# mims-harvard/Raindrop

Measured on AMD Instinct MI355X. Metric: samples/sec fwd+bwd, P19 34-sensor batch=256; % HBM roofline on msg-pass kernel, higher is better.
Workload: dtype f32

## Files before the change

### raindrop_amd/csrc/rd_attnfuse.hip

```cpp
#include <stdlib.h>

#include "rd_common.h"
#include "rd_plan.h"
#include "rd_rng.h"

namespace rd {
namespace {

typedef __bf16 bf8 __attribute__((ext_vector_type(8)));
typedef __bf16 bf4 __attribute__((ext_vector_type(4)));
typedef short sh4 __attribute__((ext_vector_type(4)));
typedef short sh8 __attribute__((ext_vector_type(8)));

constexpr int TS = 64;
constexpr int LDT = TS;
__device__ __forceinline__ int tsw(int row) { return (row & 3) | (((row >> 3) & 1) << 2); }
__device__ __forceinline__ int tofs(int row, int col) { return row * LDT + ((((col >> 3) ^ tsw(row)) & 7) << 3) + (col & 7); }
constexpr int AF_WV = 8, AF_THR = 64 * AF_WV;

struct FAttnArgs {
  const float* x;
  const __bf16* wf;
  const __bf16* wb;
  const float* bias;
  float* out; float* lse;
  const float* dout; const float* ds1; float* dx;
  __bf16* xt; __bf16* dt;
  const int32_t* plan;
  int T, B, D, H, hd;
  float scale, p_drop; uint64_t seed; uint32_t site; const uint64_t* seed_cell;
  int one;
  unsigned long long* stamps;
};
static unsigned long long* g_af_stamps = nullptr;
#define AFSTAMP(i)                                                                                  \
  do {                                                                                              \
    if (a.stamps && blockIdx.x == 0 && threadIdx.x == 0) a.stamps[(i)] = clock64();                 \
  } while (0)

__device__ __forceinline__ float g16_max(float v) {
#define RD_ROR(v, n) __builtin_bit_cast(float, __builtin_amdgcn_update_dpp(0, __builtin_bit_cast(int, v), 0x120 + (n), 0xf, 0xf, false))
  v = fmaxf(v, RD_ROR(v, 8)); v = fmaxf(v, RD_ROR(v, 4)); v = fmaxf(v, RD_ROR(v, 2)); v = fmaxf(v, RD_ROR(v, 1));
  return v;
}
__device__ __forceinline__ float g16_sum(float v) {
  v += RD_ROR(v, 8); v += RD_ROR(v, 4); v += RD_ROR(v, 2); v += RD_ROR(v, 1);
#undef RD_ROR
  return v;
}

__device__ __forceinline__ bf8 frag_n(const __bf16* P, int ld, int row0, int k0, int lane) {
  return *reinterpret_cast<const bf8*>(P + (row0 + (lane & 15)) * ld + k0 + 8 * (lane >> 4));
}
__device__ __forceinline__ bf8 frag_t(const __bf16* P, int ld, int k0, int col0, int lane) {
  const int i = lane & 15, G = lane >> 4;
  const __bf16* src = P + (k0 + 8 * G + (i >> 2)) * ld + col0 + 4 * (i & 3);
  const sh4 lo = __builtin_amdgcn_ds_read_tr16_b64_v4i16((sh4 __attribute__((address_space(3)))*)(src));
  const sh4 hi = __builtin_amdgcn_ds_read_tr16_b64_v4i16((sh4 __attribute__((address_space(3)))*)(src + 4 * ld));
  const sh8 o = {lo[0], lo[1], lo[2], lo[3], hi[0], hi[1], hi[2], hi[3]};
  return __builtin_bit_cast(bf8, o);
}
__device__ __forceinline__ bf8 frag_ns(const __bf16* P, int row0, int k0, int lane) {
  return *reinterpret_cast<const bf8*>(P + tofs(row0 + (lane & 15), k0 + 8 * (lane >> 4)));
}
__device__ __forceinline__ bf8 frag_ts(const __bf16* P, int k0, int col0, int lane) {
  const int i = lane & 15, G = lane >> 4;
  const int row = k0 + 8 * G + (i >> 2), col = col0 + 4 * (i & 3);
  const __bf16* src = P + tofs(row, col);
  const sh4 lo = __builtin_amdgcn_ds_read_tr16_b64_v4i16((sh4 __attribute__((address_space(3)))*)(src));
  const sh4 hi = __builtin_amdgcn_ds_read_tr16_b64_v4i16((sh4 __attribute__((address_space(3)))*)(src + 4 * LDT));
  const sh8 o = {lo[0], lo[1], lo[2], lo[3], hi[0], hi[1], hi[2], hi[3]};
  return __builtin_bit_cast(bf8, o);
}
template <int NT, bool AT, bool BT, bool ASW, bool BSW>
__device__ __forceinline__ void mma_b16(f32x4 (&acc)[NT], const __bf16* Ah, const __bf16* Al, int lda, int a0, const __bf16* Bh,
                                        const __bf16* Bl, int ldb, int b0, int KK, int lane, bool one) {
  auto fa = [&](const __bf16* P, int k0) {
    if (ASW) return AT ? frag_ts(P, k0, a0, lane) : frag_ns(P, a0, k0, lane);
    return AT ? frag_t(P, lda, k0, a0, lane) : frag_n(P, lda, a0, k0, lane);
  };
  auto fb = [&](const __bf16* P, int k0, int j) {
    if (BSW) return BT ? frag_ts(P, k0, b0 + 16 * j, lane) : frag_ns(P, b0 + 16 * j, k0, lane);
    return BT ? frag_t(P, ldb, k0, b0 + 16 * j, lane) : frag_n(P, ldb, b0 + 16 * j, k0, lane);
  };
  if (!one) {
#pragma unroll
    for (int k0 = 0; k0 < KK; k0 += 32) {
      const bf8 ah = fa(Ah, k0);
      const bf8 al = fa(Al, k0);
      bf8 bh[NT], bl[NT];
#pragma unroll
      for (int j = 0; j < NT; ++j) { bh[j] = fb(Bh, k0, j); bl[j] = fb(Bl, k0, j); }
#pragma unroll
      for (int j = 0; j < NT; ++j) acc[j] = __builtin_amdgcn_mfma_f32_16x16x32_bf16(al, bh[j], acc[j], 0, 0, 0);
#pragma unroll
      for (int j = 0; j < NT; ++j) acc[j] = __builtin_amdgcn_mfma_f32_16x16x32_bf16(ah, bl[j], acc[j], 0, 0, 0);
#pragma unroll
      for (int j = 0; j < NT; ++j) acc[j] = __builtin_amdgcn_mfma_f32_16x16x32_bf16(ah, bh[j], acc[j], 0, 0, 0);
    }
  } else {
#pragma unroll
    for (int k0 = 0; k0 < KK; k0 += 32) {
      const bf8 ah = fa(Ah, k0);
#pragma unroll
      for (int j = 0; j < NT; ++j) {
        const bf8 bh = fb(Bh, k0, j);
        acc[j] = __builtin_amdgcn_mfma_f32_16x16x32_bf16(ah, bh, acc[j], 0, 0, 0);
      }
    }
  }
}

__device__ __forceinline__ void split4(const float (&v)[4], bf4& hi, bf4& lo) {
#pragma unroll
  for (int r = 0; r < 4; ++r) { hi[r] = (__bf16)v[r]; lo[r] = (__bf16)(v[r] - (float)hi[r]); }
}
__device__ __forceinline__ void store_t4(__bf16* Ph, __bf16* Pl, int row, int col4, const float (&v)[4]) {
  bf4 hi, lo;
  split4(v, hi, lo);
  const int o = tofs(row, col4);
  *reinterpret_cast<bf4*>(Ph + o) = hi;
  *reinterpret_cast<bf4*>(Pl + o) = lo;
}

__device__ __forceinline__ uint64_t attn_quad(int bh, int T, int q, int key) { return ((uint64_t)bh * T + key) * ((T + 3) >> 2) + (q >> 2); }
__device__ __forceinline__ void attn_keep4(float (&k4)[4], uint64_t seed, uint32_t site, int bh, int T, int q0, int key, float p, float inv_keep) {
  const float4 u = uniform4(seed, site, attn_quad(bh, T, q0, key));
  k4[0] = u.x >= p ? inv_keep : 0.f; k4[1] = u.y >= p ? inv_keep : 0.f;
  k4[2] = u.z >= p ? inv_keep : 0.f; k4[3] = u.w >= p ? inv_keep : 0.f;
}

template <int KCX>
struct XRows { float4 v[(TS * 8 * KCX) / AF_THR]; };

template <int KCX>
__device__ __forceinline__ void x_request(XRows<KCX>& r, const float* x, long row0, int Tv, int D, int tid) {
  constexpr int kq = 8 * KCX, NIT = (TS * kq) / AF_THR;
  static_assert((TS * kq) % AF_THR == 0, "x tile must divide over the workgroup");
#pragma unroll
  for (int it = 0; it < NIT; ++it) {
    const int i = tid + it * AF_THR;
    const int rr = i / kq, k = 4 * (i - rr * kq);
    r.v[it] = *reinterpret_cast<const float4*>(x + (row0 + min(rr, Tv - 1)) * D + min(k, D - 4));
  }
}
template <int KCX>
__device__ __forceinline__ void x_store(const XRows<KCX>& r, __bf16* Xh, __bf16* Xl, int Tv, int D, int tid) {
  constexpr int kq = 8 * KCX, NIT = (TS * kq) / AF_THR, LDX = 32 * KCX + 16;
#pragma unroll
  for (int it = 0; it < NIT; ++it) {
    const int i = tid + it * AF_THR;
    const int rr = i / kq, k = 4 * (i - rr * kq);
    const bool ok = rr < Tv && k < D;
    const float v[4] = {ok ? r.v[it].x : 0.f, ok ? r.v[it].y : 0.f, ok ? r.v[it].z : 0.f, ok ? r.v[it].w : 0.f};
    bf4 hi, lo;
    split4(v, hi, lo);
    *reinterpret_cast<bf4*>(Xh + rr * LDX + k) = hi;
    *reinterpret_cast<bf4*>(Xl + rr * LDX + k) = lo;
  }
}

template <int KCX>
struct QkvPanel { bf8 h[2][KCX], l[2][KCX]; float bs[2]; };

template <int NTH, int KCX>
__device__ __forceinline__ void qkv_request(QkvPanel<KCX>& p, const __bf16* wf_h, const float* bias, int D, int hd, int h, int wave, int lane) {
  constexpr int NCT3 = 3 * NTH;
  static_assert(NCT3 <= 2 * AF_WV, "two column tiles per wave");
#pragma unroll
  for (int s = 0; s < 2; ++s) {
    const int ct = min(wave + AF_WV * s, NCT3 - 1);
    const __bf16* t = wf_h + (size_t)ct * (KCX * 2 * 512) + lane * 8;
#pragma unroll
    for (int kc = 0; kc < KCX; ++kc) {
      p.h[s][kc] = *reinterpret_cast<const bf8*>(t + (kc * 2 + 0) * 512);
      p.l[s][kc] = *reinterpret_cast<const bf8*>(t + (kc * 2 + 1) * 512);
    }
    const int whc = ct / NTH, cl = 16 * (ct - whc * NTH) + (lane & 15);
    p.bs[s] = bias[whc * D + h * hd + min(cl, hd - 1)];
  }
}

template <int NTH, int KCX>
__device__ __forceinline__ void qkv_project(const QkvPanel<KCX>& p, const __bf16* Xh, const __bf16* Xl, int hd, int Tv, __bf16* Tp, int wave,
                                            int lane, bool one) {
  constexpr int NCT3 = 3 * NTH, HDP = 32 * ((16 * NTH + 31) / 32), LDX = 32 * KCX + 16;
  const bool two = wave + AF_WV < NCT3;
  const int aoff = (lane & 15) * LDX + 8 * (lane >> 4);
  f32x4 acc[2][4];
#pragma unroll
  for (int s = 0; s < 2; ++s)
#pragma unroll
    for (int rt = 0; rt < 4; ++rt) acc[s][rt] = (f32x4){0.f, 0.f, 0.f, 0.f};
  if (!one) {
#pragma unroll
    for (int kc = 0; kc < KCX; ++kc) {
      bf8 ah[4], al[4];
#pragma unroll
      for (int rt = 0; rt < 4; ++rt) {
        ah[rt] = *reinterpret_cast<const bf8*>(Xh + rt * 16 * LDX + aoff + kc * 32);
        al[rt] = *reinterpret_cast<const bf8*>(Xl + rt * 16 * LDX + aoff + kc * 32);
      }
#pragma unroll
      for (int s = 0; s < 2; ++s)
#pragma unroll
        for (int rt = 0; rt < 4; ++rt) acc[s][rt] = __builtin_amdgcn_mfma_f32_16x16x32_bf16(al[rt], p.h[s][kc], acc[s][rt], 0, 0, 0);
#pragma unroll
      for (int s = 0; s < 2; ++s)
#pragma unroll
        for (int rt = 0; rt < 4; ++rt) acc[s][rt] = __builtin_amdgcn_mfma_f32_16x16x32_bf16(ah[rt], p.l[s][kc], acc[s][rt], 0, 0, 0);
#pragma unroll
      for (int s = 0; s < 2; ++s)
#pragma unroll
        for (int rt = 0; rt < 4; ++rt) acc[s][rt] = __builtin_amdgcn_mfma_f32_16x16x32_bf16(ah[rt], p.h[s][kc], acc[s][rt], 0, 0, 0);
    }
  } else {
#pragma unroll
    for (int kc = 0; kc < KCX; ++kc) {
#pragma unroll
      for (int rt = 0; rt < 4; ++rt) {
        const bf8 ah = *reinterpret_cast<const bf8*>(Xh + rt * 16 * LDX + aoff + kc * 32);
#pragma unroll
        for (int s = 0; s < 2; ++s) acc[s][rt] = __builtin_amdgcn_mfma_f32_16x16x32_bf16(ah, p.h[s][kc], acc[s][rt], 0, 0, 0);
      }
    }
  }
#pragma unroll
  for (int s = 0; s < 2; ++s) {
    if (s == 1 && !two) break;
    const int ct = wave + AF_WV * s;
    const int whc = ct / NTH, cl = 16 * (ct - whc * NTH) + (lane & 15);
    __bf16* Ph = Tp + (size_t)(whc * 2) * HDP * LDT;
    __bf16* Pl = Ph + (size_t)HDP * LDT;
    const bool cok = cl < hd;
#pragma unroll
    for (int rt = 0; rt < 4; ++rt) {
      const int r0 = 16 * rt + 4 * (lane >> 4);
      float v[4];
#pragma unroll
      for (int r = 0; r < 4; ++r) v[r] = (cok && r0 + r < Tv) ? acc[s][rt][r] + p.bs[s] : 0.f;
      store_t4(Ph, Pl, cl, r0, v);
    }
  }
}

template <int NTH>
__device__ __forceinline__ void zero_pad_rows(__bf16* Tp, int tid) {
  constexpr int HDP = 32 * ((16 * NTH + 31) / 32), PADR = HDP - 16 * NTH;
  if (PADR == 0) return;
  constexpr int Q8 = LDT / 4;
  for (int i = tid; i < 6 * PADR * Q8; i += AF_THR) {
    const int pl = i / (PADR * Q8), rem = i - pl * (PADR * Q8);
    const int rr = rem / Q8, q = rem - rr * Q8;
    bf4 z;
#pragma unroll
    for (int c = 0; c < 4; ++c) z[c] = (__bf16)0.f;
    *reinterpret_cast<bf4*>(Tp + ((size_t)pl * HDP + 16 * NTH + rr) * LDT + 4 * q) = z;
  }
}

template <int NTH, int KCX, bool ONE, bool SAVE = true>
__global__ __launch_bounds__(AF_THR) void k_attn_fwd_fused(FAttnArgs a) {
  extern __shared__ __attribute__((aligned(16))) unsigned char fsm[];
  RD_TOUCH_CODE(SAVE ? (ONE ? RD_TL_ATTN_FWD_B : RD_TL_ATTN_FWD) : (ONE ? RD_TL_ATTN_INF_B : RD_TL_ATTN_INF));
  constexpr int HDP = 32 * ((16 * NTH + 31) / 32), LDX = 32 * KCX + 16, NA = (NTH + 1) / 2;
  constexpr int LDO = 16 * NTH + 4;
  __bf16* Xh = reinterpret_cast<__bf16*>(fsm);
  __bf16* Xl = Xh + TS * LDX;
  __bf16* Tp = Xl + TS * LDX;
  __bf16 *Qh = Tp, *Ql = Qh + HDP * LDT, *Kh = Ql + HDP * LDT, *Kl = Kh + HDP * LDT, *Vh = Kl + HDP * LDT, *Vl = Vh + HDP * LDT;
  float* mxs = reinterpret_cast<float*>(Vl + HDP * LDT);
  float* sms = mxs + 2 * TS;
  __bf16 *Ph = Qh, *Pl = Ql;
  float* ost = reinterpret_cast<float*>(Kh);
  static_assert(HDP >= TS, "P^T must fit inside the Q^T plane");
  static_assert((size_t)TS * LDO * 4 <= (size_t)2 * HDP * LDT * 2, "output stage must fit inside the K^T planes");
  const int tid = threadIdx.x, lane = tid & 63, wave = __builtin_amdgcn_readfirstlane(tid >> 6), wq = wave & 3, wh = wave >> 2;
  const int b = blockIdx.x;
  const int Tv = __builtin_amdgcn_readfirstlane(a.plan[plan::len_base(a.B) + b]);
  if (Tv <= 0) return;
  const long row0 = __builtin_amdgcn_readfirstlane(a.plan[plan::off_base() + b]);
  uint64_t seedv = a.seed;
  XRows<KCX> xr;
  x_request<KCX>(xr, a.x, row0, Tv, a.D, tid);
  QkvPanel<KCX> pan;
  qkv_request<NTH, KCX>(pan, a.wf, a.bias, a.D, a.hd, 0, wave, lane);
  __builtin_amdgcn_sched_barrier(0);
  if (a.p_drop > 0.f && a.seed_cell) seedv += load_uniform_u64(a.seed_cell);
  zero_pad_rows<NTH>(Tp, tid);
  AFSTAMP(0);
  x_store<KCX>(xr, Xh, Xl, Tv, a.D, tid);
  AFSTAMP(1);
  lds_barrier();
  AFSTAMP(2);
  const float inv_keep = 1.0f / (1.0f - a.p_drop);
  constexpr bool one = ONE;
  const int qr0 = wq * 16 + 4 * (lane >> 4);
  for (int h = 0; h < a.H; ++h) {
    const int bh = b * a.H + h;
    if (h > 0) zero_pad_rows<NTH>(Tp, tid);
    qkv_project<NTH, KCX>(pan, Xh, Xl, a.hd, Tv, Tp, wave, lane, one);
    __builtin_amdgcn_sched_barrier(0);
    {
      const int hn = h + 1 < a.H ? h + 1 : 0;
      qkv_request<NTH, KCX>(pan, a.wf + (size_t)hn * (3 * NTH * KCX * 2 * 512), a.bias, a.D, a.hd, hn, wave, lane);
    }
    __builtin_amdgcn_sched_barrier(0);
    AFSTAMP(3 + 8 * h);
    lds_barrier();
    AFSTAMP(4 + 8 * h);
    float kp[2][4];
#pragma unroll
    for (int j = 0; j < 2; ++j)
      attn_keep4(kp[j], seedv, a.site, bh, a.T, qr0, min(16 * (2 * wh + j) + (lane & 15), a.T - 1), a.p_drop, inv_keep);
    f32x4 s[2];
#pragma unroll
    for (int j = 0; j < 2; ++j) s[j] = (f32x4){0.f, 0.f, 0.f, 0.f};
    mma_b16<2, true, true, true, true>(s, Qh, Ql, LDT, wq * 16, Kh, Kl, LDT, 32 * wh, HDP, lane, one);
    float mx[4] = {-INFINITY, -INFINITY, -INFINITY, -INFINITY};
#pragma unroll
    for (int j = 0; j < 2; ++j) {
      const int key = 16 * (2 * wh + j) + (lane & 15);
      const bool dead = key >= Tv;
#pragma unroll
      for (int r = 0; r < 4; ++r) {
        s[j][r] = dead ? -INFINITY : s[j][r] * a.scale;
        mx[r] = fmaxf(mx[r], s[j][r]);
      }
    }
#pragma unroll
    for (int r = 0; r < 4; ++r) {
      mx[r] = g16_max(mx[r]);
      if ((lane & 15) == 0) mxs[wh * TS + qr0 + r] = mx[r];
    }
    AFSTAMP(5 + 8 * h);
    lds_barrier();
    float m_i[4], rsum[4] = {0.f, 0.f, 0.f, 0.f};
#pragma unroll
    for (int r = 0; r < 4; ++r) m_i[r] = fmaxf(mxs[qr0 + r], mxs[TS + qr0 + r]);
#pragma unroll
    for (int j = 0; j < 2; ++j) {
      const int key = 16 * (2 * wh + j) + (lane & 15);
      float pv[4];
#pragma unroll
      for (int r = 0; r < 4; ++r) {
        const float p = (s[j][r] == -INFINITY) ? 0.f : __expf(s[j][r] - m_i[r]);
        rsum[r] += p;
        pv[r] = p * kp[j][r];
      }
      store_t4(Ph, Pl, key, qr0, pv);
    }
#pragma unroll
    for (int r = 0; r < 4; ++r) {
      rsum[r] = g16_sum(rsum[r]);
      if ((lane & 15) == 0) sms[wh * TS + qr0 + r] = rsum[r];
    }
    AFSTAMP(6 + 8 * h);
    lds_barrier();
    AFSTAMP(7 + 8 * h);
    float l_i[4];
#pragma unroll
    for (int r = 0; r < 4; ++r) l_i[r] = sms[qr0 + r] + sms[TS + qr0 + r];
    const int t0 = wh * NA;
    f32x4 o[NA];
#pragma unroll
    for (int j = 0; j < NA; ++j) o[j] = (f32x4){0.f, 0.f, 0.f, 0.f};
    mma_b16<NA, true, false, true, true>(o, Ph, Pl, LDT, wq * 16, Vh, Vl, LDT, 16 * t0, TS, lane, one);
#pragma unroll
    for (int r = 0; r < 4; ++r) {
      const int q = qr0 + r;
      const float inv = 1.0f / l_i[r];
#pragma unroll
      for (int j = 0; j < NA; ++j)
        if (t0 + j < NTH) ost[q * LDO + 16 * (t0 + j) + (lane & 15)] = o[j][r] * inv;
      if constexpr (SAVE) {
        if (wh == 0 && (lane & 15) == 0 && q < Tv) a.lse[(long)bh * a.T + q] = m_i[r] + logf(l_i[r]);
      }
    }
    AFSTAMP(8 + 8 * h);
    lds_barrier();
    AFSTAMP(9 + 8 * h);
    {
      const int qpr = a.hd >> 2;
      for (int e = tid; e < Tv * qpr; e += AF_THR) {
        const int q = e / qpr, c4 = e - q * qpr;
        *reinterpret_cast<float4*>(a.out + (row0 + q) * a.D + h * a.hd + 4 * c4) = *reinterpret_cast<const float4*>(ost + q * LDO + 4 * c4);
      }
    }
    lds_barrier();
    AFSTAMP(10 + 8 * h);
  }
}

template <int NTH, int KCX>
constexpr size_t fwd_lds() {
  constexpr int HDP = 32 * ((16 * NTH + 31) / 32), LDX = 32 * KCX + 16;
  return (size_t)2 * TS * LDX * 2 + (size_t)6 * HDP * LDT * 2 + (size_t)4 * TS * 4;
}

template <int NTH>
struct HRegs { float4 v[(4 * NTH + 7) / 8]; unsigned ok; };
template <int NTH>
__device__ __forceinline__ void head_request(HRegs<NTH>& h, const float* base, long ld, int Tv, int hd, int tl) {
  constexpr int NCH = (4 * NTH + 7) / 8;
  const int t = tl >> 3;
  const bool rok = t < Tv;
  const float* src = base + (long)(rok ? t : 0) * ld;
  unsigned ok = 0;
#pragma unroll
  for (int i = 0; i < NCH; ++i) {
    const int c = 4 * ((tl & 7) + 8 * i);
    const bool cok = c < hd;
    h.v[i] = *reinterpret_cast<const float4*>(src + (cok ? c : 0));
    if (rok && cok) ok |= 1u << i;
  }
  h.ok = ok;
}
template <int NTH>
__device__ __forceinline__ void head_mask(HRegs<NTH>& h) {
  constexpr int NCH = (4 * NTH + 7) / 8;
#pragma unroll
  for (int i = 0; i < NCH; ++i)
    if (!((h.ok >> i) & 1u)) h.v[i] = make_float4(0.f, 0.f, 0.f, 0.f);
}

template <int KB>
struct DxPanel { bf8 h[2][KB], l[2][KB]; };

template <int KCX, int KB, int NS>
__device__ __forceinline__ void dx_request(DxPanel<KB>& p, const __bf16* wb_h, int which, int wave, int lane) {
  constexpr int NCT = 2 * KCX;
#pragma unroll
  for (int s = 0; s < NS; ++s) {
    const __bf16* t = wb_h + ((size_t)which * NCT + wave + AF_WV * s) * (KB * 2 * 512) + lane * 8;
#pragma unroll
    for (int kc = 0; kc < KB; ++kc) {
      p.h[s][kc] = *reinterpret_cast<const bf8*>(t + (kc * 2 + 0) * 512);
      p.l[s][kc] = *reinterpret_cast<const bf8*>(t + (kc * 2 + 1) * 512);
    }
  }
}
template <int NTH, int KB, int NS, bool ONE>
__device__ __forceinline__ void dx_mma(f32x4 (&dxa)[2][4], const DxPanel<KB>& p, const __bf16* Tp, int which, int lane) {
  constexpr int HDP = 32 * ((16 * NTH + 31) / 32);
  const __bf16* Ah = Tp + (size_t)(which * 2) * HDP * LDT;
  const __bf16* Al = Ah + (size_t)HDP * LDT;
#pragma unroll
  for (int kc = 0; kc < KB; ++kc) {
    bf8 ah[4], al[4];
#pragma unroll
    for (int rt = 0; rt < 4; ++rt) {
      ah[rt] = frag_ts(Ah, 32 * kc, 16 * rt, lane);
      if (!ONE) al[rt] = frag_ts(Al, 32 * kc, 16 * rt, lane);
    }
    if (!ONE) {
#pragma unroll
      for (int s = 0; s < NS; ++s)
#pragma unroll
        for (int rt = 0; rt < 4; ++rt) dxa[s][rt] = __builtin_amdgcn_mfma_f32_16x16x32_bf16(al[rt], p.h[s][kc], dxa[s][rt], 0, 0, 0);
#pragma unroll
      for (int s = 0; s < NS; ++s)
#pragma unroll
        for (int rt = 0; rt < 4; ++rt) dxa[s][rt] = __builtin_amdgcn_mfma_f32_16x16x32_bf16(ah[rt], p.l[s][kc], dxa[s][rt], 0, 0, 0);
    }
#pragma unroll
    for (int s = 0; s < NS; ++s)
#pragma unroll
      for (int rt = 0; rt < 4; ++rt) dxa[s][rt] = __builtin_amdgcn_mfma_f32_16x16x32_bf16(ah[rt], p.h[s][kc], dxa[s][rt], 0, 0, 0);
  }
}
template <int NTH, int KCX, int NS, bool ONE>
__device__ __forceinline__ void dx_phase(f32x4 (&dxa)[2][4], DxPanel<(16 * NTH + 31) / 32>& p0, const __bf16* Tp, const __bf16* wb_h, int wave,
                                         int lane) {
  constexpr int KB = (16 * NTH + 31) / 32;
  DxPanel<KB> p1;
  dx_request<KCX, KB, NS>(p1, wb_h, 1, wave, lane);
  __builtin_amdgcn_sched_barrier(0);
  dx_mma<NTH, KB, NS, ONE>(dxa, p0, Tp, 0, lane);
  __builtin_amdgcn_sched_barrier(0);
  dx_request<KCX, KB, NS>(p0, wb_h, 2, wave, lane);
  __builtin_amdgcn_sched_barrier(0);
  dx_mma<NTH, KB, NS, ONE>(dxa, p1, Tp, 1, lane);
  __builtin_amdgcn_sched_barrier(0);
  dx_mma<NTH, KB, NS, ONE>(dxa, p0, Tp, 2, lane);
  __builtin_amdgcn_sched_barrier(0);
}

template <int NTH, int KCX, bool ONE>
__global__ __launch_bounds__(AF_THR) void k_attn_bwd_fused(FAttnArgs a) {
  extern __shared__ __attribute__((aligned(16))) unsigned char fsm[];
  RD_TOUCH_CODE(ONE ? RD_TL_ATTN_BWD_B : RD_TL_ATTN_BWD);
  constexpr int HDP = 32 * ((16 * NTH + 31) / 32), LDX = 32 * KCX + 16, NA = (NTH + 1) / 2, KB = HDP / 32, LDB = HDP + 16;
  constexpr int NCT = 2 * KCX;
  constexpr int LDS_DX = 32 * KCX + 4;
  __bf16* Xh = reinterpret_cast<__bf16*>(fsm);
  __bf16* Xl = Xh + TS * LDX;
  __bf16 *Ph = Xh, *Pl = Ph + TS * LDT, *Sh = Pl + TS * LDT, *Sl = Sh + TS * LDT;
  float* dxs = reinterpret_cast<float*>(fsm);
  static_assert((size_t)4 * TS * LDT * 2 <= (size_t)2 * TS * LDX * 2, "score planes must fit inside the x planes");
  static_assert((size_t)TS * LDS_DX * 4 <= (size_t)2 * TS * LDX * 2, "dx stage must fit inside the x planes");
  __bf16* Tp = Xl + TS * LDX;
  __bf16 *Qh = Tp, *Ql = Qh + HDP * LDT, *Kh = Ql + HDP * LDT, *Kl = Kh + HDP * LDT, *Vh = Kl + HDP * LDT, *Vl = Vh + HDP * LDT;
  __bf16* Oh = Vl + HDP * LDT;
  __bf16* Ol = Oh + TS * LDB;
  float* lse_s = reinterpret_cast<float*>(Ol + TS * LDB);
  float* dl_s = lse_s + TS;
  const int tid = threadIdx.x, lane = tid & 63, wave = __builtin_amdgcn_readfirstlane(tid >> 6), wq = wave & 3, wh = wave >> 2;
  const int b = blockIdx.x;
  const int Tv = __builtin_amdgcn_readfirstlane(a.plan[plan::len_base(a.B) + b]);
  if (Tv <= 0) return;
  const long row0 = __builtin_amdgcn_readfirstlane(a.plan[plan::off_base() + b]);
  const int g0 = __builtin_amdgcn_readfirstlane(a.plan[plan::coff_base(a.B, a.T) + b]);
  const int ngrp = (Tv + 15) >> 4;
  const bool tail_zero = (g0 + ngrp) == __builtin_amdgcn_readfirstlane(a.plan[plan::coff_base(a.B, a.T) + a.B]) && ((g0 + ngrp) & 1);
  uint64_t seedv = a.seed;
  if (a.p_drop > 0.f && a.seed_cell) seedv += load_uniform_u64(a.seed_cell);
  const float inv_keep = 1.0f / (1.0f - a.p_drop);
  constexpr bool one = ONE;
  f32x4 dxa[2][4];
#pragma unroll
  for (int s = 0; s < 2; ++s)
#pragma unroll
    for (int rt = 0; rt < 4; ++rt) dxa[s][rt] = (f32x4){0.f, 0.f, 0.f, 0.f};
  const bool two = wave + AF_WV < NCT;
  constexpr int NQ = (TS * 8 * KCX + AF_THR - 1) / AF_THR;
  QkvPanel<KCX> pan;
  HRegs<NTH> dov, ov; float lrow;
  head_request<NTH>(dov, a.dout + row0 * a.D, a.D, Tv, a.hd, tid);
  head_request<NTH>(ov, a.out + row0 * a.D, a.D, Tv, a.hd, tid);
  lrow = a.lse[(long)(b * a.H) * a.T + min(tid >> 3, Tv - 1)];
  for (int h = 0; h < a.H; ++h) {
    const int bh = b * a.H + h;
    int tl = tid;
    asm volatile("" : "+v"(tl));
    XRows<KCX> xr;
    x_request<KCX>(xr, a.x, row0, Tv, a.D, tl);
    int lq = lane;
    asm volatile("" : "+v"(lq));
    qkv_request<NTH, KCX>(pan, a.wf + (size_t)h * (3 * NTH * KCX * 2 * 512), a.bias, a.D, a.hd, h, wave, lq);
    AFSTAMP(32 + 16 * h);
    __builtin_amdgcn_sched_barrier(0);
    if (h == 0) zero_pad_rows<NTH>(Tp, tl);
    x_store<KCX>(xr, Xh, Xl, Tv, a.D, tl);
    AFSTAMP(33 + 16 * h);
    lds_barrier();
    AFSTAMP(34 + 16 * h);
    if (h == 0) {
      const int i16 = lq & 15, g2 = (lq >> 4) & 1, sub = lq >> 5;
      const int npair = (ngrp + 1) >> 1;
      for (int t = wave; t < npair * NCT * 2; t += AF_WV) {
        const int plane = t & 1, cj = t >> 1;
        const int pr = cj / NCT, j = cj - pr * NCT;
        const int lg = 2 * pr + sub;
        const __bf16* src = (plane ? Xl : Xh) + (16 * min(lg, ngrp - 1) + 8 * g2 + (i16 >> 2)) * LDX + 16 * j + 4 * (i16 & 3);
        const sh4 lo = __builtin_amdgcn_ds_read_tr16_b64_v4i16((sh4 __attribute__((address_space(3)))*)(src));
        const sh4 hi = __builtin_amdgcn_ds_read_tr16_b64_v4i16((sh4 __attribute__((address_space(3)))*)(src + 4 * LDX));
        const sh8 o = {lo[0], lo[1], lo[2], lo[3], hi[0], hi[1], hi[2], hi[3]};
        const int gg = g0 + lg;
        if (lg < ngrp)
          *reinterpret_cast<sh8*>(a.xt + (((size_t)(gg >> 1) * NCT + j) * 2 + plane) * 512 + (32 * (gg & 1) + 16 * g2 + i16) * 8) = o;
      }
      if (tail_zero) {
        const int gg = g0 + ngrp;
        const sh8 z = {0, 0, 0, 0, 0, 0, 0, 0};
        for (int i = tid; i < NCT * 2 * 32; i += AF_THR) {
          const int slot = i & 31, jp = i >> 5;
          *reinterpret_cast<sh8*>(a.xt + ((size_t)(gg >> 1) * NCT * 2 + jp) * 512 + (32 + slot) * 8) = z;
        }
      }
    }
    {
      constexpr int NCH = (4 * NTH + 7) / 8;
      head_mask<NTH>(dov);
      head_mask<NTH>(ov);
      float d = 0.f;
#pragma unroll
      for (int i = 0; i < NCH; ++i)
        d += (dov.v[i].x * ov.v[i].x + dov.v[i].y * ov.v[i].y) + (dov.v[i].z * ov.v[i].z + dov.v[i].w * ov.v[i].w);
      d += __shfl_xor(d, 1);
      d += __shfl_xor(d, 2);
      d += __shfl_xor(d, 4);
      const int o = (tl >> 3) * LDB + 4 * (tl & 7);
#pragma unroll
      for (int i = 0; i < NCH; ++i) {
        static_assert(32 * NCH == HDP, "8 threads x NCH chunks cover exactly the padded head width (chunks >= hd arrive as zeros)");
        const float v[4] = {dov.v[i].x, dov.v[i].y, dov.v[i].z, dov.v[i].w};
        bf4 hi, lo;
        split4(v, hi, lo);
        *reinterpret_cast<bf4*>(Oh + o + 32 * i) = hi;
        *reinterpret_cast<bf4*>(Ol + o + 32 * i) = lo;
      }
      if ((tl & 7) == 0) { dl_s[tl >> 3] = d; lse_s[tl >> 3] = lrow; }
    }
    __builtin_amdgcn_sched_barrier(0);
    {
      const int hn = h + 1 < a.H ? h + 1 : 0;
      head_request<NTH>(dov, a.dout + row0 * a.D + hn * a.hd, a.D, Tv, a.hd, tl);
      head_request<NTH>(ov, a.out + row0 * a.D + hn * a.hd, a.D, Tv, a.hd, tl);
      lrow = a.lse[(long)(b * a.H + hn) * a.T + min(tl >> 3, Tv - 1)];
    }
    AFSTAMP(35 + 16 * h);
    __builtin_amdgcn_sched_barrier(0);
    qkv_project<NTH, KCX>(pan, Xh, Xl, a.hd, Tv, Tp, wave, lq, one);
    AFSTAMP(36 + 16 * h);
    lds_barrier();
    AFSTAMP(37 + 16 * h);
    int l1 = lane;
    asm volatile("" : "+v"(l1));
    const int qr1 = wq * 16 + 4 * (l1 >> 4);
    float kp[2][4];
#pragma unroll
    for (int j = 0; j < 2; ++j)
      attn_keep4(kp[j], seedv, a.site, bh, a.T, qr1, min(16 * (2 * wh + j) + (l1 & 15), a.T - 1), a.p_drop, inv_keep);
    f32x4 s[2], dp[2];
#pragma unroll
    for (int j = 0; j < 2; ++j) { s[j] = (f32x4){0.f, 0.f, 0.f, 0.f}; dp[j] = s[j]; }
    mma_b16<2, true, true, true, true>(s, Qh, Ql, LDT, wq * 16, Kh, Kl, LDT, 32 * wh, HDP, l1, one);
    mma_b16<2, false, true, false, true>(dp, Oh, Ol, LDB, wq * 16, Vh, Vl, LDT, 32 * wh, HDP, l1, one);
#pragma unroll
    for (int j = 0; j < 2; ++j) {
      const int key = 16 * (2 * wh + j) + (l1 & 15);
      const bool dead = key >= Tv;
      const float (&k4)[4] = kp[j];
      float pm[4], ds[4];
#pragma unroll
      for (int r = 0; r < 4; ++r) {
        const int row = qr1 + r;
        pm[r] = 0.f; ds[r] = 0.f;
        if (!dead && row < Tv) {
          const float p = __expf(s[j][r] * a.scale - lse_s[row]);
          pm[r] = p * k4[r];
          ds[r] = p * (dp[j][r] * k4[r] - dl_s[row]) * a.scale;
        }
      }
      store_t4(Ph, Pl, key, qr1, pm);
      store_t4(Sh, Sl, key, qr1, ds);
    }
    AFSTAMP(38 + 16 * h);
    lds_barrier();
    AFSTAMP(39 + 16 * h);
    const int t0 = wh * NA;
    int l2 = lane;
    asm volatile("" : "+v"(l2));
    f32x4 dq[NA], dk[NA], dv[NA];
#pragma unroll
    for (int j = 0; j < NA; ++j) { dq[j] = (f32x4){0.f, 0.f, 0.f, 0.f}; dk[j] = dq[j]; dv[j] = dq[j]; }
    mma_b16<NA, true, false, true, true>(dq, Sh, Sl, LDT, wq * 16, Kh, Kl, LDT, 16 * t0, TS, l2, one);
    mma_b16<NA, false, false, true, true>(dk, Sh, Sl, LDT, wq * 16, Qh, Ql, LDT, 16 * t0, TS, l2, one);
    mma_b16<NA, false, true, true, false>(dv, Ph, Pl, LDT, wq * 16, Oh, Ol, LDB, 16 * t0, TS, l2, one);
    AFSTAMP(40 + 16 * h);
    lds_barrier();
    AFSTAMP(41 + 16 * h);
    const __bf16* wb_h = a.wb + (size_t)h * (3 * NCT * KB * 2 * 512);
    DxPanel<KB> dp0;
    int ld = lane;
    asm volatile("" : "+v"(ld));
    if (two) dx_request<KCX, KB, 2>(dp0, wb_h, 0, wave, ld); else dx_request<KCX, KB, 1>(dp0, wb_h, 0, wave, ld);
    __builtin_amdgcn_sched_barrier(0);
#pragma unroll
    for (int j = 0; j < NA; ++j) {
      if (t0 + j < NTH) {
        const int f = 16 * (t0 + j) + (ld & 15), qr2 = wq * 16 + 4 * (ld >> 4);
        const float vq[4] = {dq[j][0], dq[j][1], dq[j][2], dq[j][3]};
        const float vk[4] = {dk[j][0], dk[j][1], dk[j][2], dk[j][3]};
        const float vv[4] = {dv[j][0], dv[j][1], dv[j][2], dv[j][3]};
        store_t4(Qh, Ql, f, qr2, vq);
        store_t4(Kh, Kl, f, qr2, vk);
        store_t4(Vh, Vl, f, qr2, vv);
      }
    }
    AFSTAMP(42 + 16 * h);
    lds_barrier();
    AFSTAMP(43 + 16 * h);
    {
      const int i16 = ld & 15, g2 = (ld >> 4) & 1, sub = ld >> 5;
      const int nctp = 3 * a.H * NTH;
      const int npair = (ngrp + 1) >> 1;
      for (int t = wave; t < 3 * NTH * npair * 2; t += AF_WV) {
        const int plane = t & 1, u = t >> 1;
        const int pr = u / (3 * NTH), wj = u - pr * (3 * NTH);
        const int which = wj / NTH, j = wj - which * NTH;
        const int lg = 2 * pr + sub;
        const __bf16* src = Tp + (size_t)(which * 2 + plane) * HDP * LDT + tofs(16 * j + i16, 16 * min(lg, ngrp - 1) + 8 * g2);
        const sh8 o = *reinterpret_cast<const sh8*>(src);
        const int jt = (which * a.H + h) * NTH + j;
        const int gg = g0 + lg;
        if (lg < ngrp)
          *reinterpret_cast<sh8*>(a.dt + (((size_t)(gg >> 1) * nctp + jt) * 2 + plane) * 512 + (32 * (gg & 1) + 16 * g2 + i16) * 8) = o;
      }
      if (tail_zero) {
        const int gg = g0 + ngrp;
        const sh8 z = {0, 0, 0, 0, 0, 0, 0, 0};
        for (int i = tid; i < 3 * NTH * 2 * 32; i += AF_THR) {
          const int slot = i & 31, jp = i >> 5;
          const int wj = jp >> 1, plane = jp & 1;
          const int which = wj / NTH, j = wj - which * NTH;
          const int jt = (which * a.H + h) * NTH + j;
          *reinterpret_cast<sh8*>(a.dt + (((size_t)(gg >> 1) * nctp + jt) * 2 + plane) * 512 + (32 + slot) * 8) = z;
        }
      }
    }
    AFSTAMP(44 + 16 * h);
    if (two) { if (one) dx_phase<NTH, KCX, 2, true>(dxa, dp0, Tp, wb_h, wave, ld); else dx_phase<NTH, KCX, 2, false>(dxa, dp0, Tp, wb_h, wave, ld); }
    else { if (one) dx_phase<NTH, KCX, 1, true>(dxa, dp0, Tp, wb_h, wave, ld); else dx_phase<NTH, KCX, 1, false>(dxa, dp0, Tp, wb_h, wave, ld); }
    AFSTAMP(45 + 16 * h);
  }
  float4 r4[NQ];
  {
    const int qpr = a.D >> 2;
#pragma unroll
    for (int i = 0; i < NQ; ++i) {
      const int e = tid + i * AF_THR, q = e / qpr, c4 = e - q * qpr;
      r4[i] = *reinterpret_cast<const float4*>(a.ds1 + (row0 + min(q, Tv - 1)) * a.D + 4 * c4);
    }
  }
  __builtin_amdgcn_sched_barrier(0);
#pragma unroll
  for (int s = 0; s < 2; ++s) {
    if (s == 1 && !two) break;
    const int ct = wave + AF_WV * s;
#pragma unroll
    for (int rt = 0; rt < 4; ++rt)
#pragma unroll
      for (int r = 0; r < 4; ++r) dxs[(16 * rt + 4 * (lane >> 4) + r) * LDS_DX + 16 * ct + (lane & 15)] = dxa[s][rt][r];
  }
  AFSTAMP(64);
  lds_barrier();
  {
    const int qpr = a.D >> 2;
#pragma unroll
    for (int i = 0; i < NQ; ++i) {
      const int e = tid + i * AF_THR, q = e / qpr, c4 = e - q * qpr;
      if (q < Tv) {
        const float4 s4 = *reinterpret_cast<const float4*>(dxs + q * LDS_DX + 4 * c4);
        *reinterpret_cast<float4*>(a.dx + (row0 + q) * a.D + 4 * c4) = make_float4(s4.x + r4[i].x, s4.y + r4[i].y, s4.z + r4[i].z, s4.w + r4[i].w);
      }
    }
  }
  AFSTAMP(65);
}

template <int NTH, int KCX>
constexpr size_t bwd_lds() {
  constexpr int HDP = 32 * ((16 * NTH + 31) / 32), LDX = 32 * KCX + 16, LDB = HDP + 16;
  return (size_t)2 * TS * LDX * 2 + (size_t)6 * HDP * LDT * 2 + (size_t)2 * TS * LDB * 2 + (size_t)2 * TS * 4;
}

constexpr int AF_NTH = 5, AF_KCX = 5;

}

extern "C" void rd_debug_set_attnfuse_stamps(void* p) { g_af_stamps = (unsigned long long*)p; }

bool attnfuse_ok(int T, int D, int H, int hd) {
  const char* e = getenv("RD_ATTN_FUSE");
  const bool enabled = !(e && atoi(e) == 0);
  return enabled && precision() != RD_PREC_FP32 && T <= TS && hd <= 16 * AF_NTH && hd * H == D && (D + 31) / 32 == AF_KCX && (D % 4) == 0 &&
         (hd % 4) == 0 && H >= 1 && H <= 2 && 3 * AF_NTH <= 2 * AF_WV;
}
size_t attnfuse_wf_elems(int H) { return (size_t)H * 3 * AF_NTH * AF_KCX * 2 * 512; }
size_t attnfuse_wb_elems(int H) { return (size_t)H * 3 * (2 * AF_KCX) * ((16 * AF_NTH + 31) / 32) * 2 * 512; }
int attnfuse_split_specs(const float* in_proj_w, int D, int H, int hd, void* wf, void* wb, WsplitSpec* out) {
  constexpr int KB = (16 * AF_NTH + 31) / 32;
  int n = 0;
  for (int h = 0; h < H; ++h)
    for (int which = 0; which < 3; ++which) {
      const float* W = in_proj_w + ((size_t)which * D + (size_t)h * hd) * D;
      out[n++] = WsplitSpec{W, hd, D, 0, (__bf16*)wf + ((size_t)(h * 3 + which) * AF_NTH) * (AF_KCX * 2 * 512)};
      out[n++] = WsplitSpec{W, hd, D, 1, (__bf16*)wb + ((size_t)(h * 3 + which) * (2 * AF_KCX)) * (KB * 2 * 512)};
    }
  return n;
}
int attnfuse_padded_cols(int H) { return 3 * H * 16 * AF_NTH; }
int attnfuse_nth() { return AF_NTH; }

static void fill_args(FAttnArgs& a, const float* x, const void* wf, const void* wb, const float* bias, const int32_t* plan, int T, int B,
                      int D, int H, int hd, float p_drop, uint64_t seed, uint32_t site) {
  a.x = x; a.wf = (const __bf16*)wf; a.wb = (const __bf16*)wb; a.bias = bias; a.plan = plan;
  a.T = T; a.B = B; a.D = D; a.H = H; a.hd = hd;
  a.scale = 1.0f / sqrtf((float)hd); a.p_drop = p_drop; a.seed = seed; a.site = site; a.seed_cell = seed_cell();
  a.one = precision() == RD_PREC_BF16; a.stamps = g_af_stamps;
}

int launch_attn_fused_fwd(const float* x, const void* wf, const float* bias, const int32_t* plan, int T, int B, int D, int H, int hd,
                          float p_drop, uint64_t seed, uint32_t site, float* out, float* lse, hipStream_t st, bool save) {
  if (!plan) return fail(RD_EINVAL, "fused attention: needs a token plan");
  FAttnArgs a{};
  fill_args(a, x, wf, nullptr, bias, plan, T, B, D, H, hd, p_drop, seed, site);
  a.out = out; a.lse = lse;
  constexpr size_t lds = fwd_lds<AF_NTH, AF_KCX>();
  if (!save) {
    if (a.one) { RD_LDS_ATTR((k_attn_fwd_fused<AF_NTH, AF_KCX, true, false>), lds);
                 hipLaunchKernelGGL((k_attn_fwd_fused<AF_NTH, AF_KCX, true, false>), dim3(B), dim3(AF_THR), lds, st, a); }
    else { RD_LDS_ATTR((k_attn_fwd_fused<AF_NTH, AF_KCX, false, false>), lds);
           hipLaunchKernelGGL((k_attn_fwd_fused<AF_NTH, AF_KCX, false, false>), dim3(B), dim3(AF_THR), lds, st, a); }
    return check_launch("k_attn_fwd_fused<save-free>");
  }
  if (a.one) { RD_LDS_ATTR((k_attn_fwd_fused<AF_NTH, AF_KCX, true>), lds);
               hipLaunchKernelGGL((k_attn_fwd_fused<AF_NTH, AF_KCX, true>), dim3(B), dim3(AF_THR), lds, st, a); }
  else { RD_LDS_ATTR((k_attn_fwd_fused<AF_NTH, AF_KCX, false>), lds);
         hipLaunchKernelGGL((k_attn_fwd_fused<AF_NTH, AF_KCX, false>), dim3(B), dim3(AF_THR), lds, st, a); }
  return check_launch("k_attn_fwd_fused");
}

int launch_attn_fused_bwd(const float* x, const void* wf, const void* wb, const float* bias, const int32_t* plan, int T, int B, int D, int H,
                          int hd, float p_drop, uint64_t seed, uint32_t site, const float* out, const float* lse, const float* dout,
                          const float* ds1, float* dx, void* xt, void* dt, hipStream_t st) {
  if (!plan) return fail(RD_EINVAL, "fused attention: needs a token plan");
  FAttnArgs a{};
  fill_args(a, x, wf, wb, bias, plan, T, B, D, H, hd, p_drop, seed, site);
  a.out = const_cast<float*>(out); a.lse = const_cast<float*>(lse); a.dout = dout; a.ds1 = ds1; a.dx = dx;
  a.xt = (__bf16*)xt; a.dt = (__bf16*)dt;
  constexpr size_t lds = bwd_lds<AF_NTH, AF_KCX>();
  if (a.one) { RD_LDS_ATTR((k_attn_bwd_fused<AF_NTH, AF_KCX, true>), lds);
               hipLaunchKernelGGL((k_attn_bwd_fused<AF_NTH, AF_KCX, true>), dim3(B), dim3(AF_THR), lds, st, a); }
  else { RD_LDS_ATTR((k_attn_bwd_fused<AF_NTH, AF_KCX, false>), lds);
         hipLaunchKernelGGL((k_attn_bwd_fused<AF_NTH, AF_KCX, false>), dim3(B), dim3(AF_THR), lds, st, a); }
  return check_launch("k_attn_bwd_fused");
}

}
```

### raindrop_amd/csrc/rd_touch_gen.h

```cpp
#pragma once
#define RD_TL_K1_FWD_P19 13056
#define RD_TL_K1_BWD_P19 10368
#define RD_TL_K1_FWD 16640
#define RD_TL_K1_BWD 11648
#define RD_TL_ATTN_FWD 12800
#define RD_TL_ATTN_BWD 26368
#define RD_TL_ATTN_FWD_B 11136
#define RD_TL_ATTN_BWD_B 19968
#define RD_TL_EF_POST_P19L 41856
#define RD_TL_EF_POST_P19L_B 38272
#define RD_TL_EF_POST_P19 41472
#define RD_TL_EF_POST_P19_B 37888
#define RD_TL_EF_POST_P12L 41344
#define RD_TL_EF_POST_P12L_B 37760
#define RD_TL_EF_POST_P12 40960
#define RD_TL_EF_POST_P12_B 37376
#define RD_TL_EF_POST_RTL 53376
#define RD_TL_EF_POST_RTL_B 49792
#define RD_TL_EF_POST_RT 56320
#define RD_TL_EF_POST_RT_B 52736
#define RD_TL_EF_PRE_P19L 43776
#define RD_TL_EF_PRE_P19L_B 40320
#define RD_TL_EF_PRE_P19 43392
#define RD_TL_EF_PRE_P19_B 39936
#define RD_TL_EF_PRE_P12L 43264
#define RD_TL_EF_PRE_P12L_B 39936
#define RD_TL_EF_PRE_P12 42880
#define RD_TL_EF_PRE_P12_B 39552
#define RD_TL_EF_PRE_RTL 59648
#define RD_TL_EF_PRE_RTL_B 55936
#define RD_TL_EF_PRE_RT 59264
#define RD_TL_EF_PRE_RT_B 55552
#define RD_TL_K1_INF_P19 10752
#define RD_TL_ATTN_INF 11904
#define RD_TL_ATTN_INF_B 10240
#define RD_TL_EF_INF_P19 35712
#define RD_TL_EF_INF_P19_B 32128
#define RD_TL_DW 7424
#define RD_TL_DW_REDUCE 9984
#define RD_TL_ADAM 2944
#define RD_TL_ADAM_DEV 3072
#define RD_TL_WSPLIT 5248
#define RD_TL_TWG 10496
#define RD_TL_TWG_ONE 8832
#define RD_TL_HEAD_P19 15616
#define RD_TL_HEAD 17152
#define RD_TL_GEMM 26368
#define RD_TL_GEMM_X3 30080
#define RD_TL_GEMM_PANEL 33024
#define RD_TL_GEMM_PANEL_WIDE 111232
#define RD_TL_GEMM_PANEL_PC 55552
#define RD_TL_ROWGEMM 4480
#define RD_TL_ATTN_FWD_ONE 6144
#define RD_TL_ATTN_BWD_ONE 6528
#define RD_TL_ATTN_FWD_B16 7424
#define RD_TL_ATTN_BWD_DQ 7552
#define RD_TL_ATTN_BWD_DKV 6400
#define RD_TL_ADD_LN_FWD 5632
#define RD_TL_LN_BWD_R 5632
#define RD_TL_LN_BWD_V 6656
```

Measured before the change: 816,700.

## Interleave dt tile export with dx MFMA reduction steps in fused attention backward

```diff
diff --git a/raindrop_amd/csrc/rd_attnfuse.hip b/raindrop_amd/csrc/rd_attnfuse.hip
--- a/raindrop_amd/csrc/rd_attnfuse.hip
+++ b/raindrop_amd/csrc/rd_attnfuse.hip
@@ -440,9 +440,36 @@
     }
   }
 }
-template <int NTH, int KB, int NS, bool ONE>
-__device__ __forceinline__ void dx_mma(f32x4 (&dxa)[2][4], const DxPanel<KB>& p, const __bf16* Tp, int which, int lane) {
+template <int NTH>
+struct DtExport { __bf16* dt; int ngrp, g0, nctp, jt0; };
+struct DtJob { int which, j, plane, lg; };
+template <int NTH>
+__device__ __forceinline__ DtJob dt_job(const DtExport<NTH>& x, int e, int wave, int lane) {
+  const int t = wave + AF_WV * e;
+  const int u = t >> 1, pr = u / (3 * NTH), wj = u - pr * (3 * NTH);
+  const int which = wj / NTH;
+  return DtJob{which, wj - which * NTH, t & 1, min(2 * pr + (lane >> 5), x.ngrp - 1)};
+}
+template <int NTH>
+__device__ __forceinline__ sh8 dt_read(const DtExport<NTH>& x, const __bf16* Tp, int e, int wave, int lane) {
   constexpr int HDP = 32 * ((16 * NTH + 31) / 32);
+  const DtJob q = dt_job<NTH>(x, e, wave, lane);
+  return *reinterpret_cast<const sh8*>(Tp + (size_t)(q.which * 2 + q.plane) * HDP * LDT +
+                                       tofs(16 * q.j + (lane & 15), 16 * q.lg + 8 * ((lane >> 4) & 1)));
+}
+template <int NTH>
+__device__ __forceinline__ void dt_write(const DtExport<NTH>& x, int e, int wave, int lane, const sh8& v) {
+  const DtJob q = dt_job<NTH>(x, e, wave, lane);
+  const int gg = x.g0 + q.lg, jt = q.which * (x.nctp / 3) + x.jt0 + q.j;
+  *reinterpret_cast<sh8*>(x.dt + (((size_t)(gg >> 1) * x.nctp + jt) * 2 + q.plane) * 512 + (32 * (gg & 1) + (lane & 31)) * 8) = v;
+}
+
+template <int NTH, int KB, int NS, bool ONE, int E0>
+__device__ __forceinline__ void dx_mma(f32x4 (&dxa)[2][4], const DxPanel<KB>& p, const __bf16* Tp, int which, const DtExport<NTH>& x,
+                                       int wave, int lane) {
+  constexpr int HDP = 32 * ((16 * NTH + 31) / 32);
+  constexpr int DT_JOBS = (3 * NTH * 2 * (TS / 32) + AF_WV - 1) / AF_WV;
+  static_assert(DT_JOBS <= 3 * KB, "one export job per reduction step of the three products");
   const __bf16* Ah = Tp + (size_t)(which * 2) * HDP * LDT;
   const __bf16* Al = Ah + (size_t)HDP * LDT;
 #pragma unroll
@@ -453,6 +480,9 @@
       ah[rt] = frag_ts(Ah, 32 * kc, 16 * rt, lane);
       if (!ONE) al[rt] = frag_ts(Al, 32 * kc, 16 * rt, lane);
     }
+    const bool exp = E0 + kc < DT_JOBS;
+    sh8 ev;
+    if (exp) ev = dt_read<NTH>(x, Tp, E0 + kc, wave, lane);
     if (!ONE) {
 #pragma unroll
       for (int s = 0; s < NS; ++s)
@@ -467,22 +497,23 @@
     for (int s = 0; s < NS; ++s)
 #pragma unroll
       for (int rt = 0; rt < 4; ++rt) dxa[s][rt] = __builtin_amdgcn_mfma_f32_16x16x32_bf16(ah[rt], p.h[s][kc], dxa[s][rt], 0, 0, 0);
+    if (exp) dt_write<NTH>(x, E0 + kc, wave, lane, ev);
   }
 }
 template <int NTH, int KCX, int NS, bool ONE>
-__device__ __forceinline__ void dx_phase(f32x4 (&dxa)[2][4], DxPanel<(16 * NTH + 31) / 32>& p0, const __bf16* Tp, const __bf16* wb_h, int wave,
-                                         int lane) {
+__device__ __forceinline__ void dx_phase(f32x4 (&dxa)[2][4], DxPanel<(16 * NTH + 31) / 32>& p0, const __bf16* Tp, const __bf16* wb_h,
+                                         const DtExport<NTH>& x, int wave, int lane) {
   constexpr int KB = (16 * NTH + 31) / 32;
   DxPanel<KB> p1;
   dx_request<KCX, KB, NS>(p1, wb_h, 1, wave, lane);
   __builtin_amdgcn_sched_barrier(0);
-  dx_mma<NTH, KB, NS, ONE>(dxa, p0, Tp, 0, lane);
+  dx_mma<NTH, KB, NS, ONE, 0>(dxa, p0, Tp, 0, x, wave, lane);
   __builtin_amdgcn_sched_barrier(0);
   dx_request<KCX, KB, NS>(p0, wb_h, 2, wave, lane);
   __builtin_amdgcn_sched_barrier(0);
-  dx_mma<NTH, KB, NS, ONE>(dxa, p1, Tp, 1, lane);
+  dx_mma<NTH, KB, NS, ONE, KB>(dxa, p1, Tp, 1, x, wave, lane);
   __builtin_amdgcn_sched_barrier(0);
-  dx_mma<NTH, KB, NS, ONE>(dxa, p0, Tp, 2, lane);
+  dx_mma<NTH, KB, NS, ONE, 2 * KB>(dxa, p0, Tp, 2, x, wave, lane);
   __builtin_amdgcn_sched_barrier(0);
 }
 
@@ -672,37 +703,22 @@
     AFSTAMP(42 + 16 * h);
     lds_barrier();
     AFSTAMP(43 + 16 * h);
-    {
-      const int i16 = ld & 15, g2 = (ld >> 4) & 1, sub = ld >> 5;
-      const int nctp = 3 * a.H * NTH;
-      const int npair = (ngrp + 1) >> 1;
-      for (int t = wave; t < 3 * NTH * npair * 2; t += AF_WV) {
-        const int plane = t & 1, u = t >> 1;
-        const int pr = u / (3 * NTH), wj = u - pr * (3 * NTH);
+    const int nctp = 3 * a.H * NTH;
+    if (tail_zero) {
+      const int gg = g0 + ngrp;
+      const sh8 z = {0, 0, 0, 0, 0, 0, 0, 0};
+      for (int i = tid; i < 3 * NTH * 2 * 32; i += AF_THR) {
+        const int slot = i & 31, jp = i >> 5;
+        const int wj = jp >> 1, plane = jp & 1;
         const int which = wj / NTH, j = wj - which * NTH;
-        const int lg = 2 * pr + sub;
-        const __bf16* src = Tp + (size_t)(which * 2 + plane) * HDP * LDT + tofs(16 * j + i16, 16 * min(lg, ngrp - 1) + 8 * g2);
-        const sh8 o = *reinterpret_cast<const sh8*>(src);
         const int jt = (which * a.H + h) * NTH + j;
-        const int gg = g0 + lg;
-        if (lg < ngrp)
-          *reinterpret_cast<sh8*>(a.dt + (((size_t)(gg >> 1) * nctp + jt) * 2 + plane) * 512 + (32 * (gg & 1) + 16 * g2 + i16) * 8) = o;
-      }
-      if (tail_zero) {
-        const int gg = g0 + ngrp;
-        const sh8 z = {0, 0, 0, 0, 0, 0, 0, 0};
-        for (int i = tid; i < 3 * NTH * 2 * 32; i += AF_THR) {
-          const int slot = i & 31, jp = i >> 5;
-          const int wj = jp >> 1, plane = jp & 1;
-          const int which = wj / NTH, j = wj - which * NTH;
-          const int jt = (which * a.H + h) * NTH + j;
-          *reinterpret_cast<sh8*>(a.dt + (((size_t)(gg >> 1) * nctp + jt) * 2 + plane) * 512 + (32 + slot) * 8) = z;
-        }
-      }
-    }
+        *reinterpret_cast<sh8*>(a.dt + (((size_t)(gg >> 1) * nctp + jt) * 2 + plane) * 512 + (32 + slot) * 8) = z;
+      }
+    }
+    const DtExport<NTH> dte{a.dt, ngrp, g0, nctp, h * NTH};
     AFSTAMP(44 + 16 * h);
-    if (two) { if (one) dx_phase<NTH, KCX, 2, true>(dxa, dp0, Tp, wb_h, wave, ld); else dx_phase<NTH, KCX, 2, false>(dxa, dp0, Tp, wb_h, wave, ld); }
-    else { if (one) dx_phase<NTH, KCX, 1, true>(dxa, dp0, Tp, wb_h, wave, ld); else dx_phase<NTH, KCX, 1, false>(dxa, dp0, Tp, wb_h, wave, ld); }
+    if (two) { if (one) dx_phase<NTH, KCX, 2, true>(dxa, dp0, Tp, wb_h, dte, wave, ld); else dx_phase<NTH, KCX, 2, false>(dxa, dp0, Tp, wb_h, dte, wave, ld); }
+    else { if (one) dx_phase<NTH, KCX, 1, true>(dxa, dp0, Tp, wb_h, dte, wave, ld); else dx_phase<NTH, KCX, 1, false>(dxa, dp0, Tp, wb_h, dte, wave, ld); }
     AFSTAMP(45 + 16 * h);
   }
   float4 r4[NQ];
diff --git a/raindrop_amd/csrc/rd_touch_gen.h b/raindrop_amd/csrc/rd_touch_gen.h
--- a/raindrop_amd/csrc/rd_touch_gen.h
+++ b/raindrop_amd/csrc/rd_touch_gen.h
@@ -4,9 +4,9 @@
 #define RD_TL_K1_FWD 16640
 #define RD_TL_K1_BWD 11648
 #define RD_TL_ATTN_FWD 12800
-#define RD_TL_ATTN_BWD 26368
+#define RD_TL_ATTN_BWD 29056
 #define RD_TL_ATTN_FWD_B 11136
-#define RD_TL_ATTN_BWD_B 19968
+#define RD_TL_ATTN_BWD_B 22784
 #define RD_TL_EF_POST_P19L 41856
 #define RD_TL_EF_POST_P19L_B 38272
 #define RD_TL_EF_POST_P19 41472
```

Result: no change. 823,100, median of 4 (+0.8%).
